# daisy9542/yolo-puncture

Measured on AMD Instinct MI355X. Metric: images/sec, higher is better.
Workload: dtype bf16

## Files before the change

### yolo-puncture_amd/csrc/pwsp.hip

```cpp
#include "common.h"
#include <cstdlib>
#include <algorithm>

namespace yp {

typedef __attribute__((ext_vector_type(8))) __bf16 bf16x8;
typedef __attribute__((ext_vector_type(4))) float f32x4;
typedef __attribute__((ext_vector_type(4))) unsigned u32x4;
typedef __attribute__((address_space(3))) void lds_void;
typedef float f32x2 __attribute__((ext_vector_type(2)));
typedef short short2v __attribute__((ext_vector_type(2)));

__device__ __forceinline__ unsigned ps_key2(unsigned d) {
    const unsigned s = (d >> 15) & 0x00010001u;
    return d ^ ((s << 15) - s);
}
__device__ __forceinline__ uint4 ps_key4(const uint4 v) { return make_uint4(ps_key2(v.x), ps_key2(v.y), ps_key2(v.z), ps_key2(v.w)); }
__device__ __forceinline__ unsigned ps_max2(unsigned a, unsigned b) {
    const short2v r = __builtin_elementwise_max(__builtin_bit_cast(short2v, a), __builtin_bit_cast(short2v, b));
    return __builtin_bit_cast(unsigned, r);
}
__device__ __forceinline__ uint4 ps_max4(const uint4 a, const uint4 b) { return make_uint4(ps_max2(a.x, b.x), ps_max2(a.y, b.y), ps_max2(a.z, b.z), ps_max2(a.w, b.w)); }
__device__ __forceinline__ float ps_silu(float x) { return x * __builtin_amdgcn_rcpf(1.0f + __builtin_amdgcn_exp2f(x * -1.4426950408889634f)); }

__device__ unsigned long long g_ps_clk[32];
#define PS_STAMP(i) do { if (blockIdx.x == 0 && tid == 0) g_ps_clk[i] = __builtin_readcyclecounter(); } while (0)
hipError_t pwsp_read_clocks(unsigned long long* out32) { return hipMemcpyFromSymbol(out32, HIP_SYMBOL(g_ps_clk), 32 * sizeof(unsigned long long)); }

constexpr int PS_MF = 2;
constexpr int PS_NW = 16;
constexpr int PS_NT = PS_NW * 64;

template <int NS, int SP>
__global__ __launch_bounds__(PS_NT) void pwsp_kernel(const PwSpParams p) {
    constexpr int FN = NS / 16;
    constexpr int BK = 64, NSLOT = 3;
    constexpr int W_INSTR = NS / 8;
    constexpr int SLOT = W_INSTR * 1024;
    constexpr unsigned OOB = 0x80000000u;
    constexpr int KS = SP == 1 ? 3 : SP == 2 ? 7 : 1, PAD = KS / 2;
    constexpr int PIX = SP == 3 ? NS * 2 : NS * 2 + 8;
    constexpr int DW_NP = NS / 2, DW_G = PS_NT / DW_NP;
    constexpr int DW_PH = NS == 64 ? 5 : 3, DW_PW = 3;
    static_assert(SP != 3 || NS == 32, "the pool form keeps 64-byte pixel rows");

    extern __shared__ __attribute__((aligned(1024))) unsigned char smem[];
    unsigned char* const dump = smem + NSLOT * SLOT;
    unsigned char* const img = smem + NSLOT * SLOT + 1024;

    const int tid = threadIdx.x, lane = tid & 63;
    const int wave = __builtin_amdgcn_readfirstlane(tid >> 6);
    const int fr = lane & 15, fc = lane >> 4;
    const int HW = p.H * p.W;
    const int nsl = p.C1 / NS;

    int b, sl;
    {
        const int bid = blockIdx.x, nwg = gridDim.x;
        if ((p.B & 7) == 0) { const int xcd = bid & 7, j = bid >> 3; b = (j / nsl) * 8 + xcd; sl = j % nsl; }
        else { b = bid / nsl; sl = bid % nsl; }
        (void)nwg;
    }
    PS_STAMP(0);
    const int n0 = sl * NS;
    const bool spatial = SP != 0 && n0 >= p.sp_c0 && n0 + NS <= p.sp_c0 + p.Csp;
    const int nk = (p.Kpad1 + BK - 1) / BK;
    const __amdgpu_buffer_rsrc_t wrs = __builtin_amdgcn_make_buffer_rsrc((void*)p.w1, 0, (int)p.w1_bytes, 0x00020000);

    const int dgx = (p.W + DW_PW - 1) / DW_PW, dgy = (p.H + DW_PH - 1) / DW_PH;
    const int IW = (SP == 1 || SP == 2) ? dgx * DW_PW + 2 * PAD : p.W, IH = (SP == 1 || SP == 2) ? dgy * DW_PH + 2 * PAD : p.H;
    constexpr int PXS = 256 * 128;
    unsigned char* const wring = smem;
    unsigned char* const pxa = img;
    unsigned char* const pxb = img + 2 * PXS;
    const int nmf = (HW + 15) >> 4;
    const __amdgpu_buffer_rsrc_t xrs = __builtin_amdgcn_make_buffer_rsrc((void*)p.x, 0, (int)p.x_bytes, 0x00020000);
    unsigned pa_off[2], pb_off[2];
    int p_kc[2], w_kc;
#pragma unroll
    for (int j = 0; j < 2; ++j) {
        const int row = (wave * 2 + j) * 8 + (lane >> 3);
        const int c = (lane & 7) ^ ((row >> 1) & 7);
        p_kc[j] = c * 8;
        pa_off[j] = (row < HW && row < 256) ? (unsigned)((b * HW + row) * p.x_stride + p.x_coff + c * 8) * 2u : OOB;
        pb_off[j] = (row + 256 < HW) ? (unsigned)((b * HW + row + 256) * p.x_stride + p.x_coff + c * 8) * 2u : OOB;
    }
    unsigned wconst;
    {
        const int s_ = wave * 64 + lane;
        const int row = s_ >> 3, pc = s_ & 7;
        const int c = pc ^ ((row >> 1) & 7);
        w_kc = c * 8;
        wconst = (wave < W_INSTR) ? (unsigned)(((n0 + row) * p.Kpad1 + c * 8) * 2) : OOB;
    }
    auto kbyte = [&](int kt) { return (unsigned)(kt * BK) * 2u; };
    auto issue_A = [&](int kt) {
        const bool live = kt < nk;
        const unsigned kb = kbyte(kt);
        __builtin_amdgcn_raw_ptr_buffer_load_lds(wrs, (lds_void*)((wave < W_INSTR) ? wring + (kt % NSLOT) * SLOT + wave * 1024 : dump), 16,
                                                 (live && wconst != OOB && kt * BK + w_kc < p.K) ? wconst + kb : OOB, 0, 0, 0);
#pragma unroll
        for (int j = 0; j < 2; ++j)
            __builtin_amdgcn_raw_ptr_buffer_load_lds(xrs, (lds_void*)(pxa + (kt & 1) * PXS + (wave * 2 + j) * 1024), 16,
                                                     (live && pa_off[j] != OOB && kt * BK + p_kc[j] < p.K && !(p.dbg & 2)) ? pa_off[j] + kb : OOB, 0, 0, 0);
    };
    auto issue_B = [&](int kt) {
        const bool live = kt < nk;
        const unsigned kb = kbyte(kt);
#pragma unroll
        for (int j = 0; j < 2; ++j)
            __builtin_amdgcn_raw_ptr_buffer_load_lds(xrs, (lds_void*)(pxb + (kt & 1) * PXS + (wave * 2 + j) * 1024), 16,
                                                     (live && pb_off[j] != OOB && kt * BK + p_kc[j] < p.K && !(p.dbg & 2)) ? pb_off[j] + kb : OOB, 0, 0, 0);
    };

    f32x4 acc[FN][PS_MF];
#pragma unroll
    for (int a = 0; a < FN; ++a) {
        const float4 b4 = *(const float4*)(p.bias1 + n0 + a * 16 + fc * 4);
#pragma unroll
        for (int f = 0; f < PS_MF; ++f) acc[a][f] = f32x4{b4.x, b4.y, b4.z, b4.w};
    }
    const bool hasA = wave < nmf, hasB = wave + 16 < nmf;
    issue_A(0); issue_B(0); issue_A(1);
    PS_STAMP(1);
    const unsigned fro = (unsigned)(fr * 128), frs = (unsigned)((fr >> 1) & 7);
    for (int g = 0; g < nk; ++g) {
        if (g < 16) PS_STAMP(8 + g);
        __builtin_amdgcn_s_waitcnt(5 | (7 << 4) | (0xF << 8));
        __builtin_amdgcn_s_barrier();
        issue_B(g + 1);
        const unsigned char* ws = wring + (g % NSLOT) * SLOT;
        bf16x8 wf[2][FN];
#pragma unroll
        for (int s_ = 0; s_ < 2; ++s_)
#pragma unroll
            for (int a = 0; a < FN; ++a) wf[s_][a] = *(const bf16x8*)(ws + a * 2048 + fro + (((unsigned)(s_ * 4 + fc) ^ frs) << 4));
        if (hasA && !(p.dbg & 1)) {
            const unsigned char* ps = pxa + (g & 1) * PXS + wave * 2048;
#pragma unroll
            for (int s_ = 0; s_ < 2; ++s_) {
                const bf16x8 xf = *(const bf16x8*)(ps + fro + (((unsigned)(s_ * 4 + fc) ^ frs) << 4));
#pragma unroll
                for (int a = 0; a < FN; ++a) acc[a][0] = __builtin_amdgcn_mfma_f32_16x16x32_bf16(wf[s_][a], xf, acc[a][0], 0, 0, 0);
            }
        }
        __builtin_amdgcn_s_waitcnt(5 | (7 << 4) | (0xF << 8));
        __builtin_amdgcn_s_barrier();
        issue_A(g + 2);
        if (hasB && !(p.dbg & 1)) {
            const unsigned char* ps = pxb + (g & 1) * PXS + wave * 2048;
#pragma unroll
            for (int s_ = 0; s_ < 2; ++s_) {
                const bf16x8 xf = *(const bf16x8*)(ps + fro + (((unsigned)(s_ * 4 + fc) ^ frs) << 4));
#pragma unroll
                for (int a = 0; a < FN; ++a) acc[a][1] = __builtin_amdgcn_mfma_f32_16x16x32_bf16(wf[s_][a], xf, acc[a][1], 0, 0, 0);
            }
        }
    }
    __builtin_amdgcn_s_waitcnt(0 | (7 << 4) | (0xF << 8));
    __syncthreads();
    if (SP == 1 || SP == 2) {
        if (spatial) {
            const int n16 = (IH * IW * PIX + 15) >> 4;
            for (int i = tid; i < n16; i += PS_NT) *(uint4*)(img + (size_t)i * 16) = make_uint4(0, 0, 0, 0);
            __syncthreads();
        }
    }

    PS_STAMP(2);
#pragma unroll
    for (int f = 0; f < PS_MF; ++f) {
        const int m = (wave + PS_NW * f) * 16 + fr;
        const bool ok = m < HW;
        const int py = ok ? m / p.W : 0, px = ok ? m - py * p.W : 0;
#pragma unroll
        for (int a = 0; a < FN; ++a) {
            float v[4] = {acc[a][f][0], acc[a][f][1], acc[a][f][2], acc[a][f][3]};
            if (p.act1 == ACT_SILU) silu4_packed(v);
            const int co = a * 16 + fc * 4;
            if (SP == 0 && p.res1 && ok) {
                const uint2 rr = *(const uint2*)((const __bf16*)p.res1 + (size_t)(b * HW + m) * p.res1_stride + p.res1_coff + n0 + co);
                v[0] += __uint_as_float(rr.x << 16); v[1] += __uint_as_float(rr.x & 0xffff0000u);
                v[2] += __uint_as_float(rr.y << 16); v[3] += __uint_as_float(rr.y & 0xffff0000u);
            }
            __attribute__((aligned(8))) __bf16 o[4] = {(__bf16)v[0], (__bf16)v[1], (__bf16)v[2], (__bf16)v[3]};
            if (ok && p.y1) *(uint2*)((__bf16*)p.y1 + (size_t)(b * HW + m) * p.y1_stride + p.y1_coff + n0 + co) = *(const uint2*)o;
            if (SP != 0 && ok && spatial) *(uint2*)(img + (size_t)((py + PAD) * IW + px + PAD) * PIX + co * 2) = *(const uint2*)o;
        }
    }
    PS_STAMP(3);
    if (SP == 0) return;
    if (!spatial || (p.dbg & 4)) return;
    __syncthreads();
    PS_STAMP(4);

    const int cs0 = n0 - p.sp_c0;
    if constexpr (SP == 1 || SP == 2) {
        typedef __attribute__((address_space(3))) const unsigned* lds_u32p;
        typedef __attribute__((address_space(3))) const f32x2* lds_f2p;
        typedef __attribute__((address_space(3))) f32x2* lds_f2w;
        const int cp = tid % DW_NP, grp = tid / DW_NP;
        const int c = cs0 + cp * 2;
        const unsigned img_l = (unsigned)(size_t)(__attribute__((address_space(3))) unsigned char*)img;
        const unsigned wl_l = img_l + (unsigned)(((IH * IW * PIX) + 15) & ~15);
        f32x2 wk[KS == 3 ? 9 : 1];
        if constexpr (KS == 3) {
#pragma unroll
            for (int t = 0; t < 9; ++t) {
                const unsigned d = *(const unsigned*)((const __bf16*)p.wd + (size_t)t * p.Csp + c);
                wk[t] = f32x2{__uint_as_float(d << 16), __uint_as_float(d & 0xffff0000u)};
            }
        } else {
            for (int t = tid; t < KS * KS * DW_NP; t += PS_NT) {
                const unsigned d = *(const unsigned*)((const __bf16*)p.wd + (size_t)(t / DW_NP) * p.Csp + cs0 + (t % DW_NP) * 2);
                *(lds_f2w)(size_t)(wl_l + (unsigned)t * 8u) = f32x2{__uint_as_float(d << 16), __uint_as_float(d & 0xffff0000u)};
            }
            __syncthreads();
        }
        const f32x2 bias = f32x2{p.biasd[c], p.biasd[c + 1]};
        const int npatch = dgx * dgy;
        for (int q = grp; q < npatch; q += DW_G) {
            const int qy = q / dgx, qx = q - qy * dgx;
            const int oy0 = qy * DW_PH, ox0 = qx * DW_PW;
            f32x2 o[DW_PH][DW_PW];
#pragma unroll
            for (int i = 0; i < DW_PH; ++i)
#pragma unroll
                for (int j = 0; j < DW_PW; ++j) o[i][j] = bias;
            unsigned rowa = img_l + (unsigned)((oy0 * IW + ox0) * PIX + cp * 4);
#pragma unroll
            for (int r = 0; r < DW_PH + KS - 1; ++r) {
                unsigned wa = wl_l + (unsigned)cp * 8u;
                asm volatile("" : "+v"(wa));
                f32x2 xin[DW_PW + KS - 1];
#pragma unroll
                for (int cc = 0; cc < DW_PW + KS - 1; ++cc) {
                    const unsigned d = *(lds_u32p)(size_t)(rowa + (unsigned)(cc * PIX));
                    xin[cc] = f32x2{__uint_as_float(d << 16), __uint_as_float(d & 0xffff0000u)};
                }
#pragma unroll
                for (int i = 0; i < DW_PH; ++i) {
                    const int ky = r - i;
                    if (ky < 0 || ky >= KS) continue;
#pragma unroll
                    for (int kx = 0; kx < KS; ++kx) {
                        f32x2 w;
                        if constexpr (KS == 3) w = wk[ky * 3 + kx];
                        else w = *(lds_f2p)(size_t)(wa + (unsigned)((ky * KS + kx) * DW_NP * 8));
#pragma unroll
                        for (int j = 0; j < DW_PW; ++j) o[i][j] = __builtin_elementwise_fma(xin[j + kx], w, o[i][j]);
                    }
                }
                rowa += (unsigned)(IW * PIX);
#pragma unroll
                for (int i = 0; i < DW_PH; ++i) {
                    asm volatile("" : "+v"(o[i][0]), "+v"(o[i][1]), "+v"(o[i][2]));
                }
            }
            const unsigned pix0 = (unsigned)(b * HW + oy0 * p.W + ox0);
#pragma unroll
            for (int i = 0; i < DW_PH; ++i)
#pragma unroll
                for (int j = 0; j < DW_PW; ++j) {
                    if (oy0 + i >= p.H || ox0 + j >= p.W) continue;
                    float v0 = o[i][j][0], v1 = o[i][j][1];
                    if (p.actd == ACT_SILU) { v0 = ps_silu(v0); v1 = ps_silu(v1); }
                    const unsigned pix = pix0 + (unsigned)(i * p.W + j);
                    if (p.res) {
                        const unsigned rr = *(const unsigned*)((const __bf16*)p.res + (size_t)(pix * (unsigned)p.res_stride + (unsigned)(p.res_coff + c)));
                        v0 += __uint_as_float(rr << 16); v1 += __uint_as_float(rr & 0xffff0000u);
                    }
                    __attribute__((aligned(4))) __bf16 ob[2] = {(__bf16)v0, (__bf16)v1};
                    *(unsigned*)((__bf16*)p.y2 + (size_t)(pix * (unsigned)p.y2_stride + (unsigned)(p.y2_coff + c))) = *(const unsigned*)ob;
                }
        }
    } else if constexpr (SP == 3) {
        unsigned char* const bufA = img;
        unsigned char* const bufB = img + (size_t)HW * 64;
        unsigned char* const tmp = img + (size_t)HW * 128;
        const int items = HW * 4, W = p.W, H = p.H;
        for (int i = tid; i < items; i += PS_NT) *(uint4*)(bufA + i * 16) = ps_key4(*(const uint4*)(bufA + i * 16));
        __syncthreads();
        for (int stage = 0; stage < 3; ++stage) {
            const unsigned char* src = (stage & 1) ? bufB : bufA;
            unsigned char* dst = (stage & 1) ? bufA : bufB;
            for (int i = tid; i < items; i += PS_NT) {
                const int pxl = i >> 2, y = pxl / W, x = pxl - y * W;
                const int x0 = max(x - 2, 0), x1 = max(x - 1, 0), x3 = min(x + 1, W - 1), x4 = min(x + 2, W - 1);
                const unsigned char* row = src + (size_t)(y * W) * 64 + (i & 3) * 16;
                uint4 m = *(const uint4*)(row + x * 64);
                m = ps_max4(m, *(const uint4*)(row + x0 * 64));
                m = ps_max4(m, *(const uint4*)(row + x1 * 64));
                m = ps_max4(m, *(const uint4*)(row + x3 * 64));
                m = ps_max4(m, *(const uint4*)(row + x4 * 64));
                *(uint4*)(tmp + i * 16) = m;
            }
            __syncthreads();
            __bf16* yb = (__bf16*)p.y2 + (size_t)b * HW * p.y2_stride + p.y2_coff + stage * p.Csp + cs0;
            for (int i = tid; i < items; i += PS_NT) {
                const int pxl = i >> 2, y = pxl / W, x = pxl - y * W;
                const int y0 = max(y - 2, 0), y1 = max(y - 1, 0), y3 = min(y + 1, H - 1), y4 = min(y + 2, H - 1);
                const unsigned char* col = tmp + (size_t)x * 64 + (i & 3) * 16;
                uint4 m = *(const uint4*)(col + (size_t)(y * W) * 64);
                m = ps_max4(m, *(const uint4*)(col + (size_t)(y0 * W) * 64));
                m = ps_max4(m, *(const uint4*)(col + (size_t)(y1 * W) * 64));
                m = ps_max4(m, *(const uint4*)(col + (size_t)(y3 * W) * 64));
                m = ps_max4(m, *(const uint4*)(col + (size_t)(y4 * W) * 64));
                *(uint4*)(dst + i * 16) = m;
                *(uint4*)(yb + (size_t)pxl * p.y2_stride + (i & 3) * 8) = ps_key4(m);
            }
            __syncthreads();
        }
    }
    PS_STAMP(5);
}

static size_t pwsp_lds_bytes(const PwSpParams& p, int NS) {
    const size_t ring = (size_t)3 * (NS / 8) * 1024 + 1024;
    const size_t px = (size_t)4 * 256 * 128;
    size_t sp = 0;
    if (p.sp == 3) sp = (size_t)p.H * p.W * 64 * 3;
    else if (p.sp != 0) {
        const int pad = p.sp == 1 ? 1 : 3, PH = NS == 64 ? 5 : 3, PW = 3;
        const int IH = (p.H + PH - 1) / PH * PH + 2 * pad, IW = (p.W + PW - 1) / PW * PW + 2 * pad;
        sp = (((size_t)IH * IW * (NS * 2 + 8) + 15) & ~(size_t)15) + (p.sp == 2 ? (size_t)49 * (NS / 2) * 8 : 0);
    }
    return ring + std::max(px, sp);
}

int pwsp_slice(const PwSpParams& p) {
    if (p.sp == 3) return 32;
    static const int force = [] { const char* v = std::getenv("YOLOP_PWSP_NS"); return v ? atoi(v) : 0; }();
    if (force == 32) return 32;
    if (force == 64 && (p.C1 % 64) == 0 && (p.sp == 0 || ((p.sp_c0 % 64) == 0 && (p.Csp % 64) == 0))) return 64;
    if ((p.C1 % 64) == 0 && (p.sp == 0 || ((p.sp_c0 % 64) == 0 && (p.Csp % 64) == 0)) && (long)p.B * (p.C1 / 64) >= 96) return 64;
    return 32;
}

bool pwsp_valid(const PwSpParams& p) {
    if (p.sp < 0 || p.sp > 3) return false;
    const int NS = pwsp_slice(p);
    if ((p.C1 % NS) != 0 || (p.K % 32) != 0 || p.Kpad1 != p.K || p.K < 64) return false;
    if (p.H * p.W > 16 * PS_MF * PS_NW || p.H < 1 || p.W < 1) return false;
    if ((p.x_stride & 7) || (p.x_coff & 7) || p.x_bytes >= (1ull << 31) || p.w1_bytes >= (1ull << 31)) return false;
    if (p.y1 && ((p.y1_stride & 3) || (p.y1_coff & 3))) return false;
    if (p.res1 && (p.sp != 0 || (p.res1_stride & 3) || (p.res1_coff & 3))) return false;
    if ((p.C1 + 127) / 128 * 128 < p.C1) return false;
    if (p.sp != 0) {
        if (!p.y2 || (p.sp_c0 % NS) != 0 || (p.Csp % NS) != 0 || p.sp_c0 < 0 || p.sp_c0 + p.Csp > p.C1) return false;
        if ((p.y2_stride & 7) || (p.y2_coff & 7)) return false;
        if (p.res && ((p.res_stride & 1) || (p.res_coff & 1))) return false;
        if (p.sp == 3 && p.res) return false;
    } else if (!p.y1) return false;
    return pwsp_lds_bytes(p, NS) <= 160 * 1024;
}

const char* pwsp_kernel_name(const PwSpParams& p) {
    const int NS = pwsp_slice(p);
    static const char* n[2][4] = {{"pwsp_kernel<32,0>", "pwsp_kernel<32,1>", "pwsp_kernel<32,2>", "pwsp_kernel<32,3>"},
                                  {"pwsp_kernel<64,0>", "pwsp_kernel<64,1>", "pwsp_kernel<64,2>", "pwsp_kernel<64,3>"}};
    return n[NS == 64][p.sp];
}

template <int NS, int SP>
static hipError_t launch_pwsp_t(const PwSpParams& p, hipStream_t st) {
    const size_t sh = pwsp_lds_bytes(p, NS);
    auto kern = pwsp_kernel<NS, SP>;
    static size_t attr = 0;
    if (sh > attr && sh > 64 * 1024) {
        hipError_t e = hipFuncSetAttribute((const void*)kern, hipFuncAttributeMaxDynamicSharedMemorySize, 160 * 1024);
        if (e != hipSuccess) return e;
        attr = 160 * 1024;
    }
    hipLaunchKernelGGL(kern, dim3((unsigned)(p.B * (p.C1 / NS))), dim3(PS_NT), sh, st, p);
    return hipGetLastError();
}

hipError_t launch_pwsp(const PwSpParams& p, hipStream_t st) {
    if (!pwsp_valid(p)) return hipErrorInvalidValue;
    const int NS = pwsp_slice(p);
    if (NS == 64) {
        switch (p.sp) {
            case 0: return launch_pwsp_t<64, 0>(p, st);
            case 1: return launch_pwsp_t<64, 1>(p, st);
            case 2: return launch_pwsp_t<64, 2>(p, st);
            default: return hipErrorInvalidValue;
        }
    }
    switch (p.sp) {
        case 0: return launch_pwsp_t<32, 0>(p, st);
        case 1: return launch_pwsp_t<32, 1>(p, st);
        case 2: return launch_pwsp_t<32, 2>(p, st);
        default: return launch_pwsp_t<32, 3>(p, st);
    }
}

}
```

Before: 22520.

## Add wide 128-channel pointwise kernel splitting image rows into two halves

Adds a new pointwise-conv kernel variant that computes 128 output channels per block and splits each image into two row halves, with a one-row halo for the fused depthwise 3x3. It uses a triple-buffered LDS ring filled by async buffer loads and MFMA 16x16x32, and is enabled by default when the grid is large enough. The aim is more weight reuse per activation load while keeping enough blocks in flight. The cost is recomputing halo rows, more LDS per block, and more accumulator registers.

```diff
diff --git a/yolo-puncture_amd/csrc/pwsp.hip b/yolo-puncture_amd/csrc/pwsp.hip
--- a/yolo-puncture_amd/csrc/pwsp.hip
+++ b/yolo-puncture_amd/csrc/pwsp.hip
@@ -315,6 +315,269 @@
     PS_STAMP(5);
 }
 
+constexpr int PW_NS = 128;
+constexpr int PW_ROWS = 256;
+constexpr int PW_DW_PH = 5, PW_DW_PW = 3;
+
+__device__ __forceinline__ void pw_wait_vm(int n) {
+    switch (n) {
+        case 3: __builtin_amdgcn_s_waitcnt(3 | (7 << 4) | (0xF << 8)); break;
+        case 2: __builtin_amdgcn_s_waitcnt(2 | (7 << 4) | (0xF << 8)); break;
+        case 1: __builtin_amdgcn_s_waitcnt(1 | (7 << 4) | (0xF << 8)); break;
+        default: __builtin_amdgcn_s_waitcnt(0 | (7 << 4) | (0xF << 8)); break;
+    }
+}
+
+__host__ __device__ __forceinline__ void pw_part_rows(int H, int part, bool halo, int& y0, int& y1, int& g0, int& g1) {
+    const int h0 = (H + 1) / 2;
+    y0 = part ? h0 : 0; y1 = part ? H : h0;
+    g0 = halo ? (y0 > 0 ? y0 - 1 : 0) : y0;
+    g1 = halo ? (y1 < H ? y1 + 1 : H) : y1;
+}
+
+template <int SP>
+__global__ __launch_bounds__(PS_NT) void pwsp_kernel_wide(const PwSpParams p) {
+    constexpr int NS = PW_NS, FN = 4;
+    constexpr int BK = 64, NSLOT = 3;
+    constexpr int WSLOT = NS * 128, PSLOT = PW_ROWS * 128;
+    constexpr unsigned OOB = 0x80000000u;
+    constexpr int PIX = NS * 2 + 8;
+    constexpr int DW_NP = NS / 2, DW_G = PS_NT / DW_NP, DW_PH = PW_DW_PH, DW_PW = PW_DW_PW;
+    static_assert(SP == 0 || SP == 1, "the wide form is built for the plain 1x1 and the depthwise 3x3");
+
+    extern __shared__ __attribute__((aligned(1024))) unsigned char smem[];
+    unsigned char* const wring = smem;
+    unsigned char* const pring = smem + NSLOT * WSLOT;
+    unsigned char* const img = pring;
+
+    const int tid = threadIdx.x, lane = tid & 63;
+    const int wave = __builtin_amdgcn_readfirstlane(tid >> 6);
+    const int fr = lane & 15, fc = lane >> 4;
+    const int HW = p.H * p.W;
+    const int nsl = p.C1 / NS, per_img = 2 * nsl;
+
+    int b, u;
+    {
+        const int bid = blockIdx.x;
+        if ((p.B & 7) == 0) { const int xcd = bid & 7, j = bid >> 3; b = (j / per_img) * 8 + xcd; u = j % per_img; }
+        else { b = bid / per_img; u = bid % per_img; }
+    }
+    const int sl = u % nsl, part = u / nsl;
+    PS_STAMP(0);
+    const int n0 = sl * NS;
+    const bool spatial = SP != 0 && n0 >= p.sp_c0 && n0 + NS <= p.sp_c0 + p.Csp;
+    int y0, y1, g0, g1;
+    pw_part_rows(p.H, part, spatial, y0, y1, g0, g1);
+    const int npx = (g1 - g0) * p.W;
+    const int pix0 = b * HW + g0 * p.W;
+    const int nk = (p.K + BK - 1) / BK;
+    const __amdgpu_buffer_rsrc_t wrs = __builtin_amdgcn_make_buffer_rsrc((void*)p.w1, 0, (int)p.w1_bytes, 0x00020000);
+    const __amdgpu_buffer_rsrc_t xrs = __builtin_amdgcn_make_buffer_rsrc((void*)p.x, 0, (int)p.x_bytes, 0x00020000);
+
+    const int npc = (npx + 7) >> 3;
+    const bool hasp0 = wave < npc, hasp1 = wave + 16 < npc;
+    const int nw = 1 + (int)hasp0 + (int)hasp1;
+    unsigned w_off, x_off[2];
+    int w_kc, x_kc[2];
+    {
+        const int row = wave * 8 + (lane >> 3);
+        const int c = (lane & 7) ^ ((row >> 1) & 7);
+        w_kc = c * 8;
+        w_off = (unsigned)(((n0 + row) * p.Kpad1 + c * 8) * 2);
+    }
+#pragma unroll
+    for (int j = 0; j < 2; ++j) {
+        const int row = (wave + 16 * j) * 8 + (lane >> 3);
+        const int c = (lane & 7) ^ ((row >> 1) & 7);
+        x_kc[j] = c * 8;
+        x_off[j] = row < npx ? (unsigned)((pix0 + row) * p.x_stride + p.x_coff + c * 8) * 2u : OOB;
+    }
+    auto issue = [&](int kt) {
+        const int k0 = kt * BK;
+        const unsigned kb = (unsigned)k0 * 2u;
+        __builtin_amdgcn_raw_ptr_buffer_load_lds(wrs, (lds_void*)(wring + (kt % NSLOT) * WSLOT + wave * 1024), 16,
+                                                 k0 + w_kc < p.K ? w_off + kb : OOB, 0, 0, 0);
+        unsigned char* const ps = pring + (kt % NSLOT) * PSLOT;
+        if (hasp0)
+            __builtin_amdgcn_raw_ptr_buffer_load_lds(xrs, (lds_void*)(ps + wave * 1024), 16,
+                                                     (x_off[0] != OOB && k0 + x_kc[0] < p.K && !(p.dbg & 2)) ? x_off[0] + kb : OOB, 0, 0, 0);
+        if (hasp1)
+            __builtin_amdgcn_raw_ptr_buffer_load_lds(xrs, (lds_void*)(ps + (wave + 16) * 1024), 16,
+                                                     (x_off[1] != OOB && k0 + x_kc[1] < p.K && !(p.dbg & 2)) ? x_off[1] + kb : OOB, 0, 0, 0);
+    };
+
+    const int ch = wave & 1, pg = wave >> 1;
+    const int nmf = (npx + 15) >> 4;
+    const bool hasf0 = 2 * pg < nmf, hasf1 = 2 * pg + 1 < nmf;
+    f32x4 acc[FN][2];
+#pragma unroll
+    for (int a = 0; a < FN; ++a) {
+        const float4 b4 = *(const float4*)(p.bias1 + n0 + (ch * FN + a) * 16 + fc * 4);
+        acc[a][0] = f32x4{b4.x, b4.y, b4.z, b4.w};
+        acc[a][1] = acc[a][0];
+    }
+    issue(0);
+    if (nk > 1) issue(1);
+    PS_STAMP(1);
+    const unsigned fro = (unsigned)(fr * 128), frs = (unsigned)((fr >> 1) & 7);
+    auto kstep = [&](int g) {
+        const unsigned char* ws = wring + (g % NSLOT) * WSLOT + ch * FN * 2048;
+        const unsigned char* ps = pring + (g % NSLOT) * PSLOT + pg * 4096;
+        if (p.dbg & 1) return;
+#pragma unroll
+        for (int s_ = 0; s_ < 2; ++s_) {
+            const unsigned co = fro + (((unsigned)(s_ * 4 + fc) ^ frs) << 4);
+            bf16x8 wf[FN];
+#pragma unroll
+            for (int a = 0; a < FN; ++a) wf[a] = *(const bf16x8*)(ws + a * 2048 + co);
+            if (hasf0) {
+                const bf16x8 xf = *(const bf16x8*)(ps + co);
+#pragma unroll
+                for (int a = 0; a < FN; ++a) acc[a][0] = __builtin_amdgcn_mfma_f32_16x16x32_bf16(wf[a], xf, acc[a][0], 0, 0, 0);
+            }
+            if (hasf1) {
+                const bf16x8 xf = *(const bf16x8*)(ps + 2048 + co);
+#pragma unroll
+                for (int a = 0; a < FN; ++a) acc[a][1] = __builtin_amdgcn_mfma_f32_16x16x32_bf16(wf[a], xf, acc[a][1], 0, 0, 0);
+            }
+        }
+    };
+    for (int g = 0; g < nk - 1; ++g) {
+        if (g < 16) PS_STAMP(8 + g);
+        pw_wait_vm(nw);
+        __builtin_amdgcn_s_barrier();
+        if (g + 2 < nk) issue(g + 2);
+        kstep(g);
+    }
+    if (nk - 1 < 16) PS_STAMP(8 + nk - 1);
+    __builtin_amdgcn_s_waitcnt(0 | (7 << 4) | (0xF << 8));
+    __builtin_amdgcn_s_barrier();
+    kstep(nk - 1);
+    __syncthreads();
+
+    const int hp = y1 - y0;
+    const int dgx = (p.W + DW_PW - 1) / DW_PW, dgy = (hp + DW_PH - 1) / DW_PH;
+    const int IW = dgx * DW_PW + 2, IH = dgy * DW_PH + 2;
+    if (SP == 1 && spatial) {
+        const int n16 = (IH * IW * PIX + 15) >> 4;
+        for (int i = tid; i < n16; i += PS_NT) *(uint4*)(img + (size_t)i * 16) = make_uint4(0, 0, 0, 0);
+        __syncthreads();
+    }
+    PS_STAMP(2);
+#pragma unroll
+    for (int f = 0; f < 2; ++f) {
+        const int m = (pg * 2 + f) * 16 + fr;
+        const bool ok = m < npx;
+        const int gy = ok ? m / p.W : 0, px = ok ? m - gy * p.W : 0;
+        const int py = g0 + gy;
+        const bool own = ok && py >= y0 && py < y1;
+#pragma unroll
+        for (int a = 0; a < FN; ++a) {
+            float v[4] = {acc[a][f][0], acc[a][f][1], acc[a][f][2], acc[a][f][3]};
+            if (p.act1 == ACT_SILU) silu4_packed(v);
+            const int co = (ch * FN + a) * 16 + fc * 4;
+            if (SP == 0 && p.res1 && own) {
+                const uint2 rr = *(const uint2*)((const __bf16*)p.res1 + (size_t)(pix0 + m) * p.res1_stride + p.res1_coff + n0 + co);
+                v[0] += __uint_as_float(rr.x << 16); v[1] += __uint_as_float(rr.x & 0xffff0000u);
+                v[2] += __uint_as_float(rr.y << 16); v[3] += __uint_as_float(rr.y & 0xffff0000u);
+            }
+            __attribute__((aligned(8))) __bf16 o[4] = {(__bf16)v[0], (__bf16)v[1], (__bf16)v[2], (__bf16)v[3]};
+            if (own && p.y1) *(uint2*)((__bf16*)p.y1 + (size_t)(pix0 + m) * p.y1_stride + p.y1_coff + n0 + co) = *(const uint2*)o;
+            if (SP == 1 && ok && spatial) *(uint2*)(img + (size_t)((py - y0 + 1) * IW + px + 1) * PIX + co * 2) = *(const uint2*)o;
+        }
+    }
+    PS_STAMP(3);
+    if (SP == 0) return;
+    if (!spatial || (p.dbg & 4)) return;
+    __syncthreads();
+    PS_STAMP(4);
+
+    if constexpr (SP == 1) {
+        typedef __attribute__((address_space(3))) const unsigned* lds_u32p;
+        const int cs0 = n0 - p.sp_c0;
+        const int cp = tid % DW_NP, grp = tid / DW_NP;
+        const int c = cs0 + cp * 2;
+        const unsigned img_l = (unsigned)(size_t)(__attribute__((address_space(3))) unsigned char*)img;
+        f32x2 wk[9];
+#pragma unroll
+        for (int t = 0; t < 9; ++t) {
+            const unsigned d = *(const unsigned*)((const __bf16*)p.wd + (size_t)t * p.Csp + c);
+            wk[t] = f32x2{__uint_as_float(d << 16), __uint_as_float(d & 0xffff0000u)};
+        }
+        const f32x2 bias = f32x2{p.biasd[c], p.biasd[c + 1]};
+        const int npatch = dgx * dgy;
+        for (int q = grp; q < npatch; q += DW_G) {
+            const int qy = q / dgx, qx = q - qy * dgx;
+            const int oy0 = qy * DW_PH, ox0 = qx * DW_PW;
+            f32x2 o[DW_PH][DW_PW];
+#pragma unroll
+            for (int i = 0; i < DW_PH; ++i)
+#pragma unroll
+                for (int j = 0; j < DW_PW; ++j) o[i][j] = bias;
+            unsigned rowa = img_l + (unsigned)((oy0 * IW + ox0) * PIX + cp * 4);
+#pragma unroll
+            for (int r = 0; r < DW_PH + 2; ++r) {
+                f32x2 xin[DW_PW + 2];
+#pragma unroll
+                for (int cc = 0; cc < DW_PW + 2; ++cc) {
+                    const unsigned d = *(lds_u32p)(size_t)(rowa + (unsigned)(cc * PIX));
+                    xin[cc] = f32x2{__uint_as_float(d << 16), __uint_as_float(d & 0xffff0000u)};
+                }
+#pragma unroll
+                for (int i = 0; i < DW_PH; ++i) {
+                    const int ky = r - i;
+                    if (ky < 0 || ky >= 3) continue;
+#pragma unroll
+                    for (int kx = 0; kx < 3; ++kx)
+#pragma unroll
+                        for (int j = 0; j < DW_PW; ++j) o[i][j] = __builtin_elementwise_fma(xin[j + kx], wk[ky * 3 + kx], o[i][j]);
+                }
+                rowa += (unsigned)(IW * PIX);
+#pragma unroll
+                for (int i = 0; i < DW_PH; ++i) {
+                    asm volatile("" : "+v"(o[i][0]), "+v"(o[i][1]), "+v"(o[i][2]));
+                }
+            }
+            const unsigned pixq = (unsigned)(b * HW + (y0 + oy0) * p.W + ox0);
+#pragma unroll
+            for (int i = 0; i < DW_PH; ++i)
+#pragma unroll
+                for (int j = 0; j < DW_PW; ++j) {
+                    if (oy0 + i >= hp || ox0 + j >= p.W) continue;
+                    float v0 = o[i][j][0], v1 = o[i][j][1];
+                    if (p.actd == ACT_SILU) { v0 = ps_silu(v0); v1 = ps_silu(v1); }
+                    const unsigned pix = pixq + (unsigned)(i * p.W + j);
+                    if (p.res) {
+                        const unsigned rr = *(const unsigned*)((const __bf16*)p.res + (size_t)(pix * (unsigned)p.res_stride + (unsigned)(p.res_coff + c)));
+                        v0 += __uint_as_float(rr << 16); v1 += __uint_as_float(rr & 0xffff0000u);
+                    }
+                    __attribute__((aligned(4))) __bf16 ob[2] = {(__bf16)v0, (__bf16)v1};
+                    *(unsigned*)((__bf16*)p.y2 + (size_t)(pix * (unsigned)p.y2_stride + (unsigned)(p.y2_coff + c))) = *(const unsigned*)ob;
+                }
+        }
+    }
+    PS_STAMP(5);
+}
+
+static size_t pwsp_wide_lds_bytes(const PwSpParams& p) {
+    const size_t ring = (size_t)3 * PW_NS * 128 + (size_t)3 * PW_ROWS * 128;
+    if (p.sp != 1) return ring;
+    const int hp = (p.H + 1) / 2;
+    const size_t img = (size_t)((hp + PW_DW_PH - 1) / PW_DW_PH * PW_DW_PH + 2) * ((p.W + PW_DW_PW - 1) / PW_DW_PW * PW_DW_PW + 2) * (PW_NS * 2 + 8);
+    return (size_t)3 * PW_NS * 128 + std::max((size_t)3 * PW_ROWS * 128, (img + 15) & ~(size_t)15);
+}
+
+static bool pwsp_wide(const PwSpParams& p) {
+    static const int mode = [] { const char* v = std::getenv("YOLOP_PWSP_WIDE"); return v && *v ? atoi(v) : 1; }();
+    if (mode == 0 || (p.sp != 0 && p.sp != 1)) return false;
+    if ((p.C1 % PW_NS) != 0 || (p.K % 32) != 0 || p.Kpad1 != p.K || p.K < 64 || p.H < 2 || p.W < 1) return false;
+    if (p.sp == 1 && ((p.sp_c0 % PW_NS) != 0 || (p.Csp % PW_NS) != 0)) return false;
+    if (mode != 2 && (long)p.B * 2 * (p.C1 / PW_NS) < 192) return false;
+    const int hp = (p.H + 1) / 2;
+    if ((hp + (p.sp == 1 ? 1 : 0)) * p.W > PW_ROWS) return false;
+    return pwsp_wide_lds_bytes(p) <= 160 * 1024;
+}
+
 static size_t pwsp_lds_bytes(const PwSpParams& p, int NS) {
     const size_t ring = (size_t)3 * (NS / 8) * 1024 + 1024;
     const size_t px = (size_t)4 * 256 * 128;
@@ -332,6 +595,7 @@
     if (p.sp == 3) return 32;
     static const int force = [] { const char* v = std::getenv("YOLOP_PWSP_NS"); return v ? atoi(v) : 0; }();
     if (force == 32) return 32;
+    if (force == 0 && pwsp_wide(p)) return PW_NS;
     if (force == 64 && (p.C1 % 64) == 0 && (p.sp == 0 || ((p.sp_c0 % 64) == 0 && (p.Csp % 64) == 0))) return 64;
     if ((p.C1 % 64) == 0 && (p.sp == 0 || ((p.sp_c0 % 64) == 0 && (p.Csp % 64) == 0)) && (long)p.B * (p.C1 / 64) >= 96) return 64;
     return 32;
@@ -352,11 +616,12 @@
         if (p.res && ((p.res_stride & 1) || (p.res_coff & 1))) return false;
         if (p.sp == 3 && p.res) return false;
     } else if (!p.y1) return false;
-    return pwsp_lds_bytes(p, NS) <= 160 * 1024;
+    return (NS == PW_NS ? pwsp_wide_lds_bytes(p) : pwsp_lds_bytes(p, NS)) <= 160 * 1024;
 }
 
 const char* pwsp_kernel_name(const PwSpParams& p) {
     const int NS = pwsp_slice(p);
+    if (NS == PW_NS) return p.sp == 0 ? "pwsp_kernel_wide<0>" : "pwsp_kernel_wide<1>";
     static const char* n[2][4] = {{"pwsp_kernel<32,0>", "pwsp_kernel<32,1>", "pwsp_kernel<32,2>", "pwsp_kernel<32,3>"},
                                   {"pwsp_kernel<64,0>", "pwsp_kernel<64,1>", "pwsp_kernel<64,2>", "pwsp_kernel<64,3>"}};
     return n[NS == 64][p.sp];
@@ -376,9 +641,24 @@
     return hipGetLastError();
 }
 
+template <int SP>
+static hipError_t launch_pwsp_wide_t(const PwSpParams& p, hipStream_t st) {
+    const size_t sh = pwsp_wide_lds_bytes(p);
+    auto kern = pwsp_kernel_wide<SP>;
+    static size_t attr = 0;
+    if (sh > attr) {
+        hipError_t e = hipFuncSetAttribute((const void*)kern, hipFuncAttributeMaxDynamicSharedMemorySize, 160 * 1024);
+        if (e != hipSuccess) return e;
+        attr = 160 * 1024;
+    }
+    hipLaunchKernelGGL(kern, dim3((unsigned)(p.B * 2 * (p.C1 / PW_NS))), dim3(PS_NT), sh, st, p);
+    return hipGetLastError();
+}
+
 hipError_t launch_pwsp(const PwSpParams& p, hipStream_t st) {
     if (!pwsp_valid(p)) return hipErrorInvalidValue;
     const int NS = pwsp_slice(p);
+    if (NS == PW_NS) return p.sp == 0 ? launch_pwsp_wide_t<0>(p, st) : launch_pwsp_wide_t<1>(p, st);
     if (NS == 64) {
         switch (p.sp) {
             case 0: return launch_pwsp_t<64, 0>(p, st);
```

After: 22640 (median of 6 runs). About the same (+0.5%).
